# HBioquant/DiffBindFR

Hardware: AMD Instinct MI355X
Metric: poses_per_sec (higher is better)
Workload: dtype f32

## Files before the change

### diffbindfr_amd/csrc/api.cpp

```cpp
#include <cmath>
#include <cstdio>
#include <cstring>
#include <algorithm>
#include <atomic>
#include <map>

#include "common.h"

void launch_conv(const ConvArgs& a, hipStream_t st);
void launch_conv_layer(const ConvArgs* c4, hipStream_t st);
void launch_conv2(const Conv2Args& a, hipStream_t st);
void launch_conv2h(const Conv2Args& a, hipStream_t st);
void launch_convz(const ConvZArgs& a, hipStream_t st);
void launch_reduce_ln(const float* msg, const int* row_start, const int* row_cnt, int N, int D, const LNDesc& ln,
                      const float* old, int D_old, float* out, int ldo, int mode, hipStream_t st, const uint8_t* first = nullptr, unsigned long long sc_lanes = 0);
struct ReduceLayerArgs {
  const float* msg[4]; const int* row_start[4]; const int* row_cnt[4]; LNDesc ln[4];
  int NL, NA, D, D_old;
  const float* old_l; const float* old_a; float* out_l; float* out_a;
  const uint8_t* first[4]; unsigned long long sc_lanes[4];
};
static unsigned long long convz_sc_lanes(const ConvZ& z) {
  unsigned long long m = 0;
  for (int i = 0; i < z.n_io; ++i) m |= 0xfffull << (z.out_off[i] / 4);
// ... 5 lines not shown
  dbfr_batch b;
  const int* lig_batch; const int* atm_batch; const uint8_t* is_cab; const int* n_cab; const float* tr_sigma;
  float lig_cut2, atom_cut2, cross_cut2;
  int lig_cap, atom_cap, dynamic_cross;
  EdgeSet set[N_SETS];
  int* err;
  int step, lds_nl, lds_na, n_chunk, lanes;
};
void dbfr_edge_form(const dbfr_batch& b, int* n_chunk, int* lanes);
void launch_edges(const GraphArgs& A, bool heads_only, hipStream_t st);
void launch_edge_log(const GraphArgs& A, int* log_row, int stride, hipStream_t st);
void launch_edge_ties(const GraphArgs& A, int* log_row, int stride, float tol, hipStream_t st);
void launch_graph_chunks(const GraphArgs& A, hipStream_t st);
void launch_flat_chunks(const int* tgt, const int* n_edges, int max_edges, int span, int n_span, int* cnt0, int cap, int* chunk_es, int* chunk_gl, hipStream_t st);
void launch_row_absmax(const float* lx, const int* lig_ptr, float* out_l, const float* ax, const int* atm_ptr, float* out_a, int ld, int D, int G, int n_rows_a, hipStream_t st);
void launch_batch_vectors(const dbfr_batch& b, int* lig_batch, int* atm_batch, uint8_t* is_cab, int* n_cab,
                          int* tor_batch, int* sc_batch, hipStream_t st);
void launch_time_embed(const float* t, int G, float emb_scale, float* temb, hipStream_t st);
enum MlpIn { IN_LIGNODE = 0, IN_LIGEDGE = 1, IN_TG = 2, IN_G = 3 };
struct MlpArgs {
  Mlp2 w; int mode; const int* n_rows_dev; int n_rows_max; const float* temb; const int* row_graph_tab; const int* tgt;
  const int* aux; const float* dist; const float* bond_feat; int nfeat; const float* lig_node; int nnode;
  const float* gs_offset; const float* gs_coeff; float* out;
};
void launch_mlp(const MlpArgs& a, hipStream_t st);
struct AtomEncArgs {
  const float* pocket_feat; const int* atm_batch; const float* temb; const float* emb[5]; int dims[5];
  const float* lin_t; int NA; float* out;
};
void launch_atom_encoder(const AtomEncArgs& a, hipStream_t st);
void launch_center_edges(const dbfr_batch& b, int* tgt, int* gth, float* dist, float* sh, int* row_start, int* row_cnt,
                         hipStream_t st);
struct TrRotArgs {
  const float* gp; const float* temb; const float* tr_sigma; const float* rot_norm; Mlp2 tr, rot; int G;
  int scale_by_sigma; float* tr_out; float* rot_out; int* err;
};
void launch_trrot(const TrRotArgs& a, hipStream_t st);
void launch_bond_attr(const float* x, int ldx, const int* b0, const int* b1, const int* bsel, int stride, int n,
                      float* out, hipStream_t st);
void launch_tor_final(const float* feat, const Mlp2& w, const float* norm2, int scale, int n, float* out, hipStream_t st);
struct SdeLigArgs {
  dbfr_batch b; const float* tr_score; const float* rot_score; const float* tor_score; const float* z_tr;
  const float* z_rot; const float* z_tor; float dt, tr_g2, tr_gsdt, rot_g2, rot_gsdt, tor_g2, tor_gsdt; float* traj;
  int* err;
};
void launch_sde_ligand(const SdeLigArgs& a, hipStream_t st);
// ... 56 lines not shown

struct dbfr_model {
  dbfr_model_cfg cfg;
  std::vector<void*> allocs;
  ConvW layer[8][4];
  ConvW final_conv, tor_conv, sc_conv;
  ConvW2 layer2[8][4], tor_conv2, sc_conv2;
  ConvW2 layer2v[8][4];
  ConvZ layerz[8][4], tor_convz, sc_convz;
  int use_conv2;
  int gemm_split;
  int* queue;
  std::string fallback_convs;
  std::string rowscaled_convs;
  uint32_t layer_fallback;
  int* edge_log; int edge_log_steps, edge_log_graphs;
  int* tie_log; int tie_log_steps, tie_log_graphs; float tie_tol;
  Mlp2 lig_node_emb, lig_edge_emb, atom_edge_emb, la_edge_emb, center_edge_emb, tor_edge_emb, sc_edge_emb;
  Mlp2 tr_final, rot_final, tor_final, sc_final;
  const float* atom_emb[5]; int atom_dims[5];
  const float* atom_lin_t;
  const float *gs_lig_off, *gs_lig_c, *gs_atom_off, *gs_atom_c, *gs_cross_off, *gs_cross_c, *gs_center_off, *gs_center_c;
  int* a14_group;
  int profile;
  std::vector<hipEvent_t> ev;
  size_t ev_used;
  double* flops_dev;
  double fused_bytes_last;
  double executed_last;
  double useful_last;
  double form_bytes_last;
  double conv_ms_acc; int64_t conv_launches_acc;
};

template <typename T>
static T* upload(dbfr_model* m, const std::vector<T>& h, int* rc) {
  void* d = nullptr;
  size_t bytes = std::max<size_t>(h.size() * sizeof(T), 16);
  if (hipMalloc(&d, bytes) != hipSuccess) { *rc = DBFR_ERR_HIP; g_err = "hipMalloc failed (model weights)"; return nullptr; }
  if (!h.empty() && hipMemcpy(d, h.data(), h.size() * sizeof(T), hipMemcpyHostToDevice) != hipSuccess) {
    *rc = DBFR_ERR_HIP; g_err = "hipMemcpy failed (model weights)"; return nullptr;
  }
  m->allocs.push_back(d);
  return (T*)d;
}

typedef std::map<std::string, const dbfr_tensor*> TMap;

static const float* need(const TMap& tm, const std::string& name, int64_t numel, int* rc) {
  auto it = tm.find(name);
  if (it == tm.end()) { *rc = fail(DBFR_ERR_ARG, "missing tensor '" + name + "'"); return nullptr; }
  if (it->second->numel != numel) {
    *rc = fail(DBFR_ERR_ARG, "tensor '" + name + "' has " + std::to_string(it->second->numel) + " elements, expected " +
                                 std::to_string(numel));
    return nullptr;
  }
  return it->second->data;
}

static int pack_mlp(dbfr_model* m, const TMap& tm, const std::string& name, int in, int hid, int out, bool bias, Mlp2* o) {
  int rc = 0;
  const float* w0 = need(tm, name + ".lin.0.weight", (int64_t)hid * in, &rc);
  const float* w1 = need(tm, name + ".lin.3.weight", (int64_t)out * hid, &rc);
  const float *b0 = nullptr, *b1 = nullptr;
  if (bias) { b0 = need(tm, name + ".lin.0.bias", hid, &rc); b1 = need(tm, name + ".lin.3.bias", out, &rc); }
  if (rc) return rc;
  std::vector<float> w0t((size_t)in * hid), w1t((size_t)hid * out);
// ... 930 lines not shown
      acc(descs[i].n_edges, 2.0 * 144 * (144.0 + Ws[i]), m->flops_dev);
      acc(descs[i].n_edges, 4.0 * (Ws[i] + descs[i].w.D_in + 9) + 16.0, m->flops_dev + 1);
      acc(descs[i].n_edges, fused_bytes(descs[i].w.D_in, descs[i].w.D_out), m->flops_dev + 2);
      const double rows = 16.0 * descs[i].w.n_tiles;
      const bool f16 = (m->gemm_split >= DBFR_GEMM_SPLIT_F16 && !f16_fallback) || z;
      const double ex = f16 ? 3.0 * 2.0 * 144 * (144.0 + rows) : 2.0 * 144 * (144.0 + rows);
      if (!z || descs[i].w.n_tiles > 0) acc(descs[i].n_edges, ex, m->flops_dev + 3);
      if (!z) acc(descs[i].n_edges, ex, m->flops_dev + 4);
      else if (descs[i].w.n_tiles > 0) acc(descs[i].n_edges, 3.0 * 2.0 * 144 * rows, m->flops_dev + 4);
      const int D_in = descs[i].w.D_in, D_out = descs[i].w.D_out;
      const double in_bytes = 4.0 * (48 + 9 + 3 + 48 + 48 + D_in);
      if (!z) acc(descs[i].n_edges, fused_bytes(D_in, D_out), m->flops_dev + 5);
      else acc(descs[i].n_edges, in_bytes + 1.0 + (descs[i].w.n_tiles > 0 ? in_bytes + 4.0 * (D_out - 48 * z[i].w.n_io) : 0.0), m->flops_dev + 5);
    }
    launch_acc_batch(ab, st);
  }
}

static int run_score(dbfr_model* m, const dbfr_batch* B, const dbfr_cond* c, const dbfr_scores* out, Ws& w,
                     hipStream_t st, int step = 0) {
  const dbfr_model_cfg& cfg = m->cfg;
  const int G = B->G, NL = B->NL, NA = B->NA;
  launch_time_embed(c->t, G, cfg.emb_scale, w.temb, st);
  GraphArgs ga;
  ga.b = *B; ga.lig_batch = w.lig_batch; ga.atm_batch = w.atm_batch; ga.is_cab = w.is_cab; ga.n_cab = w.n_cab;
  ga.tr_sigma = c->tr_sigma;
  ga.lig_cut2 = cfg.lig_cutoff * cfg.lig_cutoff; ga.atom_cut2 = cfg.atom_cutoff * cfg.atom_cutoff;
  ga.cross_cut2 = cfg.dynamic_max_cross ? 1.0f : cfg.cross_cutoff * cfg.cross_cutoff;
  ga.lig_cap = cfg.lig_max_neighbors; ga.atom_cap = cfg.atom_max_neighbors; ga.dynamic_cross = cfg.dynamic_max_cross;
  for (int k = 0; k < N_SETS; ++k) ga.set[k] = w.set[k];
  ga.err = w.err; ga.step = step; ga.lds_nl = ga.lds_na = 0;
  dbfr_edge_form(*B, &ga.n_chunk, &ga.lanes);
  launch_edges(ga, false, st);
  if (int lrc = take_launch_error()) return lrc;
  if (m->gemm_split == DBFR_GEMM_REDUCE_FIRST) launch_graph_chunks(ga, st);
  if (m->edge_log && step < m->edge_log_steps) launch_edge_log(ga, m->edge_log + (size_t)step * N_SETS * m->edge_log_graphs, m->edge_log_graphs, st);
  if (m->tie_log && step < m->tie_log_steps) launch_edge_ties(ga, m->tie_log + (size_t)step * N_SETS * m->tie_log_graphs, m->tie_log_graphs, m->tie_tol, st);
  {
    MlpArgs a; memset(&a, 0, sizeof a);
    a.w = m->lig_node_emb; a.mode = IN_LIGNODE; a.n_rows_max = NL; a.temb = w.temb; a.row_graph_tab = w.lig_batch;
    a.lig_node = B->lig_node; a.nnode = cfg.lig_node_features; a.out = w.lig_x[0];
    launch_mlp(a, st);
  }
  {
    AtomEncArgs a; a.pocket_feat = B->pocket_feat; a.atm_batch = w.atm_batch; a.temb = w.temb;
    for (int i = 0; i < 5; ++i) { a.emb[i] = m->atom_emb[i]; a.dims[i] = m->atom_dims[i]; }
    a.lin_t = m->atom_lin_t; a.NA = NA; a.out = w.atom_x[0];
    launch_atom_encoder(a, st);
  }
  auto edge_mlp = [&](const Mlp2& mw, int mode, const EdgeSet& S, const int* tab, const float* off, const float* co) {
    MlpArgs a; memset(&a, 0, sizeof a);
    a.w = mw; a.mode = mode; a.n_rows_dev = S.n_edges; a.n_rows_max = S.cap; a.temb = w.temb; a.row_graph_tab = tab;
    a.tgt = S.tgt; a.aux = S.aux; a.dist = S.dist; a.bond_feat = B->bond_feat; a.nfeat = cfg.lig_edge_features;
    a.gs_offset = off; a.gs_coeff = co; a.out = S.emb;
    launch_mlp(a, st);
  };
  edge_mlp(m->lig_edge_emb, IN_LIGEDGE, w.set[SET_LL], w.lig_batch, m->gs_lig_off, m->gs_lig_c);
  edge_mlp(m->atom_edge_emb, IN_TG, w.set[SET_AA], w.atm_batch, m->gs_atom_off, m->gs_atom_c);
  edge_mlp(m->la_edge_emb, IN_TG, w.set[SET_AL], w.lig_batch, m->gs_cross_off, m->gs_cross_c);
  edge_mlp(m->la_edge_emb, IN_TG, w.set[SET_LA], w.atm_batch, m->gs_cross_off, m->gs_cross_c);
  static const int dims[4] = {48, 84, 120, 168};
  int cur = 0;
  for (int l = 0; l < cfg.num_conv_layers; ++l) {
    const int Di = dims[std::min(l, 3)], Do = dims[std::min(l + 1, 3)];
    const float *lx = w.lig_x[cur], *ax = w.atom_x[cur];
    float *lnew = w.lig_x[cur ^ 1], *anew = w.atom_x[cur ^ 1];
    const EdgeSet &LL = w.set[SET_LL], &AA = w.set[SET_AA], &AL = w.set[SET_AL], &LA = w.set[SET_LA];
    const ConvSite sites[4] = {conv_site(LL, G, lx, Di, LL.tgt, lx, Di, LL.gth, lx, Di, w.msg[0], w.xmax_l),
                               conv_site(AL, G, lx, Di, AL.tgt, ax, Di, AL.gth, ax, Di, w.msg[1], w.xmax_a),
                               conv_site(AA, G, ax, Di, AA.tgt, ax, Di, AA.gth, ax, Di, w.msg[2], w.xmax_a),
                               conv_site(LA, G, ax, Di, LA.tgt, lx, Di, LA.gth, lx, Di, w.msg[3], w.xmax_l)};
    const bool fallback = (m->layer_fallback >> l) & 1u;
    const bool rf = w.conv2 && m->gemm_split == DBFR_GEMM_REDUCE_FIRST && !fallback;
    if (w.conv2) {
      Conv2Desc ds[4]; ConvZDesc zs[4]; int Ws[4];
      for (int i = 0; i < 4; ++i) {
        ds[i] = conv2_desc(sites[i], rf ? m->layer2v[l][i] : m->layer2[l][i]);
// ... 12 lines not shown
      }
      launch_conv_layer(c4, st);
      if (m->profile == 1) (void)hipEventRecord(e1, st);
      if (m->profile)
        for (int i = 0; i < 4; ++i)
          launch_acc_flops(c4[i].n_edges, 2.0 * 144 * (144.0 + m->layer[l][i].W), 4.0 * (m->layer[l][i].W + Di + 9) + 16.0, fused_bytes(Di, Do), m->flops_dev, st);
    }
    ReduceLayerArgs ra;
    for (int i = 0; i < 4; ++i) {
      ra.msg[i] = sites[i].msg; ra.row_start[i] = sites[i].row_start; ra.row_cnt[i] = sites[i].row_cnt; ra.ln[i] = m->layer[l][i].ln;
      ra.first[i] = rf ? sites[i].seg_first : nullptr; ra.sc_lanes[i] = rf ? convz_sc_lanes(m->layerz[l][i]) : 0;
    }
    ra.NL = NL; ra.NA = NA; ra.D = Do; ra.D_old = Di; ra.old_l = lx; ra.old_a = ax; ra.out_l = lnew; ra.out_a = anew;
    launch_reduce_ln_layer(ra, st);
    cur ^= 1;
  }
  const int D = dims[std::min(cfg.num_conv_layers, 3)];
  if (D != MAXD) return fail(DBFR_ERR_ARG, "heads need num_conv_layers >= 3");
  const float *lx = w.lig_x[cur], *ax = w.atom_x[cur];
  launch_center_edges(*B, w.c_tgt, w.c_gth, w.c_dist, w.c_sh, w.c_row_start, w.c_row_cnt, st);
  {
    MlpArgs a; memset(&a, 0, sizeof a);
    a.w = m->center_edge_emb; a.mode = IN_TG; a.n_rows_max = NL; a.temb = w.temb; a.row_graph_tab = w.lig_batch;
    a.dist = w.c_dist; a.gs_offset = m->gs_center_off; a.gs_coeff = m->gs_center_c; a.out = w.c_emb;
    launch_mlp(a, st);
  }
  conv_call(m, m->final_conv, flat_site(w.n_edges6 + 7, NL, w.c_tgt, w.c_gth, w.c_emb, w.c_sh, lx, D, w.c_gth, nullptr, 0, w.c_gth, lx, D, w.msg[0]), st);
  launch_reduce_ln(w.msg[0], w.c_row_start, w.c_row_cnt, G, 12, m->final_conv.ln, nullptr, 0, w.gp, 12, 2, st);
  {
    TrRotArgs a; a.gp = w.gp; a.temb = w.temb; a.tr_sigma = c->tr_sigma; a.rot_norm = c->rot_score_norm;
    a.tr = m->tr_final; a.rot = m->rot_final; a.G = G; a.scale_by_sigma = cfg.scale_by_sigma; a.tr_out = out->tr;
    a.rot_out = out->rot; a.err = w.err;
    launch_trrot(a, st);
  }
  struct TorHead {
    bool on; int n; const EdgeSet* S; ConvSite site;
    const float* nodes; const int *b0, *b1, *bsel; int stride; float* attr;
    const Mlp2* emb; const float *gs_off, *gs_c;
    const ConvW* cw; const ConvW2* cw2; const ConvZ* cz;
    const Mlp2* fin; const float* norm2; float *feat, *out;
  };
  const EdgeSet &T = w.set[SET_TOR], &S = w.set[SET_SC];
  TorHead heads[2];
  {
    TorHead& h = heads[0];
    h.on = B->NTOR > 0; h.n = B->NTOR; h.S = &T;
    h.site = conv_site(T, G, lx, D, T.gth, w.tor_attr, NS, T.tgt, lx, D, w.msg[0], w.xmax_l);
// ... 378 lines not shown
  const ConvW* cw = pick_conv(m, layer, family);
  if (!cw) return fail(DBFR_ERR_ARG, "no such conv");
  unsigned long long lanes = 0;
  if (seg_first) {
    if (layer == -1 || cw->K != 144) return fail(DBFR_ERR_ARG, "dbfr_test_reduce_ln2: seg_first with a conv that has no reduce-first form");
    lanes = convz_sc_lanes(*pick_conv144(m, layer, family).z);
  }
  launch_reduce_ln(msg, row_start, row_cnt, n_nodes, cw->D_out, cw->ln, old, d_old, out, cw->D_out, mode, (hipStream_t)hip_stream, seg_first, lanes);
  HIPCHECK(hipGetLastError());
  return DBFR_OK;
}

extern "C" int dbfr_test_reduce_ln(dbfr_model* m, int32_t layer, int32_t family, const float* msg,
                                   const int32_t* row_start, const int32_t* row_cnt, int32_t n_nodes, const float* old,
                                   int32_t d_old, float* out, int32_t mode, void* hip_stream) {
  if (!m) return fail(DBFR_ERR_ARG, "null model");
  const ConvW* cw = pick_conv(m, layer, family);
  if (!cw) return fail(DBFR_ERR_ARG, "no such conv");
  launch_reduce_ln(msg, row_start, row_cnt, n_nodes, cw->D_out, cw->ln, old, d_old, out, cw->D_out, mode,
                   (hipStream_t)hip_stream);
  HIPCHECK(hipGetLastError());
  return DBFR_OK;
}
```

### diffbindfr_amd/csrc/conv.hip

```cpp
#include <cstdio>
#include <cstdlib>
#include <type_traits>
#include <vector>

#include "common.h"

#ifndef CONV_PRIO
#define CONV_PRIO 0
#endif
#ifndef CONV_XPF
#define CONV_XPF 0
#endif
#ifndef CONV_NB2_WAVES
#define CONV_NB2_WAVES 2
#endif
#define XS_LD (MAXD + 4)

typedef float f32x4 __attribute__((ext_vector_type(4)));

#define TRACE_BLOCKS 1024
#define TRACE_TILES 48
#define TRACE_REC (2 + 3 * TRACE_TILES + 8)
#define RSTAMP(k) do { if ((ABL & 16) && a.trace && bid < TRACE_BLOCKS && lane == 0) a.trace[((size_t)bid * 4 + wave) * TRACE_REC + 2 + 3 * TRACE_TILES + (k)] = __builtin_amdgcn_s_memrealtime(); } while (0)
#define TSTAMP(k) do { if ((ABL & 16) && a.trace && bid < TRACE_BLOCKS && lane == 0) a.trace[((size_t)bid * 4 + wave) * TRACE_REC + 2 + 3 * TRACE_TILES + (k)] = __builtin_readcyclecounter(); } while (0)
// ... 500 lines not shown
      float v = buf[wave][c];
      float* o = out + (size_t)node * ldo + c;
      if (mode == 0) v = (c < D_old ? old[(size_t)node * D_old + c] : 0.f) + v;
      else if (mode == 1) v = *o + v;
      *o = v;
    }
  }
}

void launch_reduce_ln(const float* msg, const int* row_start, const int* row_cnt, int N, int D, const LNDesc& ln,
                      const float* old, int D_old, float* out, int ldo, int mode, hipStream_t st, const uint8_t* first, unsigned long long sc_lanes) {
  if (N <= 0) return;
  hipLaunchKernelGGL(k_reduce_ln, dim3((N + 3) / 4), dim3(256), 0, st, msg, row_start, row_cnt, N, D, ln, old, D_old,
                     out, ldo, mode, first, sc_lanes);
}

struct ReduceLayerArgs {
  const float* msg[4]; const int* row_start[4]; const int* row_cnt[4]; LNDesc ln[4];
  int NL, NA, D, D_old;
  const float* old_l; const float* old_a; float* out_l; float* out_a;
  const uint8_t* first[4]; unsigned long long sc_lanes[4];
};

__device__ __forceinline__ void mean_ln(const float* __restrict__ msg, int rs, int rc, int D, const LNDesc& ln, float* bw, int lane, const uint8_t* first, unsigned long long sc_lanes) {
  const int d4 = D >> 2;
  const f32x4 acc = row_sum(msg, rs, rc, D, lane, first, sc_lanes);
  if (lane < d4) {
    const float cntf = (float)max(rc, 1);
    bw[4 * lane] = acc[0] / cntf; bw[4 * lane + 1] = acc[1] / cntf; bw[4 * lane + 2] = acc[2] / cntf; bw[4 * lane + 3] = acc[3] / cntf;
  }
  __builtin_amdgcn_wave_barrier();
  int iw = 0, ib = 0;
  for (int bk = 0; bk < ln.nblk; ++bk) {
    const int mul = ln.mul[bk], dim = ln.dim[bk], off = ln.off[bk];
    const int nel = mul * dim;
    float mean[3] = {0.f, 0.f, 0.f};
    const bool d3 = dim == 3;
    for (int i = lane; i < nel; i += 64) {
      int comp = d3 ? i % 3 : 0;
      float v = bw[off + i];
      if (comp == 0) mean[0] += v; else if (comp == 1) mean[1] += v; else mean[2] += v;
    }
    for (int o = 32; o > 0; o >>= 1) mean[0] += __shfl_xor(mean[0], o);
    mean[0] /= (float)mul;
    if (d3) {
#pragma unroll
      for (int c = 1; c < 3; ++c) {
        for (int o = 32; o > 0; o >>= 1) mean[c] += __shfl_xor(mean[c], o);
        mean[c] /= (float)mul;
      }
    }
    float sq = 0.f;
    for (int i = lane; i < nel; i += 64) {
      int u = d3 ? i / 3 : i, comp = d3 ? i - 3 * u : 0;
      float v = bw[off + i] - (comp == 0 ? mean[0] : comp == 1 ? mean[1] : mean[2]) * ln.mean_shift[iw + u];
      bw[off + i] = v;
      sq += v * v;
    }
    __builtin_amdgcn_wave_barrier();
    for (int o = 32; o > 0; o >>= 1) sq += __shfl_xor(sq, o);
    const float inv = 1.0f / sqrtf(sq / (float)nel + 1e-5f);
    for (int i = lane; i < nel; i += 64) {
      int u = d3 ? i / 3 : i;
      float v = bw[off + i] * (inv * ln.weight[iw + u]);
      if (ln.is0e[bk]) v += ln.bias[ib + u];
      bw[off + i] = v;
    }
    iw += mul;
    if (ln.is0e[bk]) ib += mul;
  }
  __builtin_amdgcn_wave_barrier();
}

__global__ __launch_bounds__(256) void k_reduce_ln_layer(ReduceLayerArgs a) {
  __shared__ float buf[4][2][MAXD];
  const int lane = threadIdx.x & 63, wave = threadIdx.x >> 6;
  const int nbl = (a.NL + 3) / 4;
  const bool lig = (int)blockIdx.x < nbl;
  const int node = (lig ? blockIdx.x : blockIdx.x - nbl) * 4 + wave;
  const int N = lig ? a.NL : a.NA;
  if (node >= N) return;
  const int s0 = lig ? 0 : 2;
  mean_ln(a.msg[s0], a.row_start[s0][node], a.row_cnt[s0][node], a.D, a.ln[s0], buf[wave][0], lane, a.first[s0], a.sc_lanes[s0]);
  mean_ln(a.msg[s0 + 1], a.row_start[s0 + 1][node], a.row_cnt[s0 + 1][node], a.D, a.ln[s0 + 1], buf[wave][1], lane, a.first[s0 + 1], a.sc_lanes[s0 + 1]);
  const float* old = (lig ? a.old_l : a.old_a) + (size_t)node * a.D_old;
  float* out = (lig ? a.out_l : a.out_a) + (size_t)node * a.D;
#pragma unroll
  for (int j = 0; j < 3; ++j) {
    const int c = lane + 64 * j;
    if (c < a.D) out[c] = ((c < a.D_old ? old[c] : 0.f) + buf[wave][0][c]) + buf[wave][1][c];
  }
}

void launch_reduce_ln_layer(const ReduceLayerArgs& a, hipStream_t st) {
  const int nb = (a.NL + 3) / 4 + (a.NA + 3) / 4;
  if (nb <= 0) return;
  hipLaunchKernelGGL(k_reduce_ln_layer, dim3(nb), dim3(256), 0, st, a);
}
```

### diffbindfr_amd/csrc/graph.hip

```cpp
#include "common.h"

#define MAX_NL 256
#define MAX_NA 8192

enum SetKind { SET_LL = 0, SET_AA = 1, SET_AL = 2, SET_LA = 3, SET_TOR = 4, SET_SC = 5, N_SETS = 6 };

struct GraphArgs {
  dbfr_batch b;
  const int* lig_batch;
  const int* atm_batch;
  const uint8_t* is_cab;
  const int* n_cab;
  const float* tr_sigma;
  float lig_cut2, atom_cut2, cross_cut2;
  int lig_cap, atom_cap, dynamic_cross;
  EdgeSet set[N_SETS];
  int* err;
  int step;
  int lds_nl, lds_na;
  int n_chunk;
  int lanes;
};

__device__ __forceinline__ float d2_rn(float ax, float ay, float az, float bx, float by, float bz) {
// ... 648 lines not shown
void launch_time_embed(const float* t, int G, float emb_scale, float* temb, hipStream_t st) {
  hipLaunchKernelGGL(k_time_embed, dim3((G * EMB + 255) / 256), dim3(256), 0, st, t, G, emb_scale, temb);
}

enum MlpIn { IN_LIGNODE = 0, IN_LIGEDGE = 1, IN_TG = 2, IN_G = 3 };

struct MlpArgs {
  Mlp2 w;
  int mode;
  const int* n_rows_dev;
  int n_rows_max;
  const float* temb;
  const int* row_graph_tab;
  const int* tgt;
  const int* aux;
  const float* dist;
  const float* bond_feat;
  int nfeat;
  const float* lig_node;
  int nnode;
  const float* gs_offset;
  const float* gs_coeff;
  float* out;
};

#define MLP_ROWS 64
#define MLP_MAXIN 80

__global__ __launch_bounds__(256) void k_mlp(MlpArgs a) {
  __shared__ float xin[MLP_ROWS][MLP_MAXIN + 1];
  __shared__ float hid[MLP_ROWS][NS + 1];
  __shared__ float w0[MLP_MAXIN * NS];
  __shared__ float w1[NS * NS];
  __shared__ float s_gs[EMB];
  const int nrows = a.n_rows_dev ? min(*a.n_rows_dev, a.n_rows_max) : a.n_rows_max;
  if ((int)blockIdx.x * MLP_ROWS >= nrows) return;
  const int in = a.w.in;
  for (int i = threadIdx.x; i < in * NS; i += 256) w0[i] = a.w.w0t[i];
  for (int i = threadIdx.x; i < NS * NS; i += 256) w1[i] = a.w.w1t[i];
  const float coeff = a.gs_coeff ? a.gs_coeff[0] : 0.f;
  if (threadIdx.x < EMB) s_gs[threadIdx.x] = a.gs_offset ? a.gs_offset[threadIdx.x] : 0.f;
  __syncthreads();
  const int kin = (in + 3) & ~3;
  if (kin > in)
    for (int i = threadIdx.x; i < (kin - in) * NS; i += 256) w0[in * NS + i] = 0.f;
  typedef float f32x4 __attribute__((ext_vector_type(4)));
// ... 47 lines not shown
  }
#pragma unroll
  for (int t = 0; t < 3; ++t)
#pragma unroll
    for (int r = 0; r < 4; ++r) hid[row][16 * t + 4 * g + r] = fmaxf(acc[t][r], 0.f);
  __syncthreads();
#pragma unroll
  for (int t = 0; t < 3; ++t)
#pragma unroll
    for (int r = 0; r < 4; ++r) acc[t][r] = a.w.b1 ? a.w.b1[16 * t + 4 * g + r] : 0.f;
#pragma unroll
  for (int k = 0; k < NS; k += 4) {
    const float bv = hid[row][k + g];
#pragma unroll
    for (int t = 0; t < 3; ++t) acc[t] = __builtin_amdgcn_mfma_f32_16x16x4f32(w1[(k + g) * NS + 16 * t + n], bv, acc[t], 0, 0, 0);
  }
  if (row < nr) {
#pragma unroll
    for (int t = 0; t < 3; ++t) *reinterpret_cast<f32x4*>(a.out + (size_t)(r0 + row) * NS + 16 * t + 4 * g) = acc[t];
  }
  }
}

void launch_mlp(const MlpArgs& a, hipStream_t st) {
  if (a.n_rows_max <= 0) return;
  const int tiles = (a.n_rows_max + MLP_ROWS - 1) / MLP_ROWS;
  hipLaunchKernelGGL(k_mlp, dim3(tiles < 1024 ? tiles : 1024), dim3(256), 0, st, a);
}

struct AtomEncArgs {
  const float* pocket_feat;
  const int* atm_batch;
  const float* temb;
  const float* emb[5];
  int dims[5];
  const float* lin_t;
  int NA;
  float* out;
};

__global__ __launch_bounds__(256) void k_atom_encoder(AtomEncArgs a) {
  __shared__ float w[(NS + EMB) * NS];
  __shared__ float x[16][NS + EMB];
  for (int i = threadIdx.x; i < (NS + EMB) * NS; i += 256) w[i] = a.lin_t[i];
  const int r0 = blockIdx.x * 16;
  for (int i = threadIdx.x; i < 16 * (NS + EMB); i += 256) {
    int r = i / (NS + EMB), c = i % (NS + EMB);
    int row = r0 + r;
// ... 30 lines not shown
```

### diffbindfr_amd/lib.py

```python
import ctypes as C
import os

HERE = os.path.dirname(os.path.abspath(__file__))
LIB_PATH = os.environ.get("DBFR_LIB") or os.path.join(HERE, "libdbfr.so")

DBFR_OK = 0
DBFR_ERR_CAPACITY = -3
ERRORS = {-1: "DBFR_ERR_ARG", -2: "DBFR_ERR_HIP", -3: "DBFR_ERR_CAPACITY", -4: "DBFR_ERR_SELFTEST",
          -5: "DBFR_ERR_NUMERIC"}

i32, f32, vp = C.c_int32, C.c_float, C.c_void_p


class ModelCfg(C.Structure):
    _fields_ = [(n, i32) for n in ("ns", "nv", "sh_lmax", "num_conv_layers", "lig_node_features",
                                   "lig_edge_features", "distance_embed_dim", "sigma_embed_dim")] + \
               [(n, f32) for n in ("emb_scale", "lig_cutoff", "atom_cutoff", "cross_cutoff", "center_max_distance")] + \
               [(n, i32) for n in ("atom_max_neighbors", "lig_max_neighbors", "dynamic_max_cross", "scale_by_sigma",
                                   "no_sc_torsion")]


class Tensor(C.Structure):
    _fields_ = [("name", C.c_char_p), ("data", vp), ("numel", C.c_int64)]

# ... 232 lines not shown

class XtcOpts(C.Structure):
    _fields_ = [("precision", f32), ("dt", f32), ("first_step", i32), ("box", f32 * 9)]


class SitesOpts(C.Structure):
    _fields_ = [(n, f32) for n in ("spacing", "probe", "ray_length", "lining_cutoff")] + \
               [(n, i32) for n in ("min_buried", "min_points", "max_sites")]


class SitesIn(C.Structure):
    _fields_ = [("n_prot", i32), ("n_res", i32), ("max_points", C.c_int64)] + \
               [(n, vp) for n in ("res_ptr", "aatype", "atom37_pos", "atom37_mask", "radius")]


class SitesOut(C.Structure):
    _fields_ = [(n, vp) for n in ("n_sites", "label", "n_points", "score", "idx_sum", "centre", "lining", "grid", "occupancy",
                                  "burial", "labels")]


SYMBOLS = ["dbfr_model_create", "dbfr_model_destroy", "dbfr_model_set_edge_log", "dbfr_model_set_tie_log", "dbfr_model_fallback_convs", "dbfr_model_rowscaled_convs", "dbfr_model_set_gemm", "dbfr_model_get_gemm", "dbfr_workspace_bytes", "dbfr_score", "dbfr_sample",
           "dbfr_sample_range", "dbfr_capacity_report",
           "dbfr_init_poses", "dbfr_extract_templates", "dbfr_status_sync", "dbfr_abi_version", "dbfr_build_id", "dbfr_last_error", "dbfr_wigner3j", "dbfr_conv_paths", "dbfr_test_pack_f16_tiles", "dbfr_test_pack_f16_rows", "dbfr_test_chunk_table", "dbfr_test_pack_f16_depth", "dbfr_probe_mfma_f16",
           "dbfr_profile_enable", "dbfr_profile_read", "dbfr_profile_fused_bytes", "dbfr_profile_executed_flops", "dbfr_profile_useful_flops", "dbfr_workspace_layout", "dbfr_test_conv", "dbfr_test_conv2", "dbfr_test_reduce_ln", "dbfr_test_reduce_ln2", "dbfr_test_sde_step",
           "dbfr_pose_metrics", "dbfr_pdb_format", "dbfr_pdb_write_files", "dbfr_select_pocket", "dbfr_sdf_format",
           "dbfr_sdf_write_files", "dbfr_mdn_model_create", "dbfr_mdn_model_destroy", "dbfr_mdn_workspace_bytes", "dbfr_mdn_forward", "dbfr_mdn_pocket_features",
           "dbfr_vina_workspace_bytes", "dbfr_vina_score", "dbfr_vina_score_at", "dbfr_vina_minimize",
           "dbfr_vina_flex_workspace_bytes", "dbfr_vina_flex_score_at", "dbfr_vina_flex_minimize",
           "dbfr_pose_rmsd_matrix", "dbfr_select_modes", "dbfr_pose_check",
           "dbfr_pdb_atom_map", "dbfr_complex_pdb_format", "dbfr_complex_pdb_write_files", "dbfr_xtc_workspace_bytes", "dbfr_xtc_encode",
           "dbfr_sites_workspace_bytes", "dbfr_find_sites", "dbfr_interactions", "dbfr_pocket_check", "dbfr_sasa",
           "dbfr_seq_align", "dbfr_holo_site", "dbfr_holo_metrics", "dbfr_hetero_check", "dbfr_hydrogens"]

_lib = None


class DbfrError(RuntimeError):
    pass


def load():
    global _lib
    if _lib is not None:
        return _lib
    if not os.path.exists(LIB_PATH):
        raise DbfrError(f"{LIB_PATH} is missing: build the HIP library first "
                        f"(python -m diffbindfr_amd.build). There is no CPU fallback.")
# ... 20 lines not shown
    lib.dbfr_init_poses.argtypes = [vp, C.POINTER(Batch), C.POINTER(InitTape), vp, vp]
    lib.dbfr_extract_templates.argtypes = [i32, vp, vp, vp, vp, vp, vp, vp, vp]
    lib.dbfr_status_sync.argtypes = [vp, vp, C.POINTER(C.c_int64)]
    lib.dbfr_wigner3j.argtypes = [i32, i32, i32, C.POINTER(C.c_double)]
    lib.dbfr_conv_paths.argtypes = [i32, C.POINTER(i32), i32, C.POINTER(i32)]
    lib.dbfr_test_pack_f16_tiles.argtypes = [vp, vp, i32, vp, C.POINTER(i32)]
    lib.dbfr_test_pack_f16_depth.argtypes = [vp, vp, i32, C.POINTER(i32), C.POINTER(i32)]
    lib.dbfr_test_pack_f16_rows.argtypes = [vp, vp, i32, vp, C.POINTER(i32), vp, C.POINTER(i32)]
    lib.dbfr_test_chunk_table.argtypes = [vp, vp, i32, i32, vp, i32, vp, vp, vp]
    lib.dbfr_probe_mfma_f16.argtypes = [C.c_double, C.POINTER(C.c_double), vp]
    lib.dbfr_profile_enable.argtypes = [vp, i32]
    lib.dbfr_profile_fused_bytes.argtypes = [vp, C.POINTER(C.c_double)]
    lib.dbfr_profile_executed_flops.argtypes = [vp, C.POINTER(C.c_double)]
    lib.dbfr_profile_useful_flops.argtypes = [vp, C.POINTER(C.c_double), C.POINTER(C.c_double)]
    lib.dbfr_profile_read.argtypes = [vp, C.POINTER(C.c_double), C.POINTER(C.c_int64), C.POINTER(C.c_double),
                                      C.POINTER(C.c_double), i32]
    lib.dbfr_workspace_layout.argtypes = [vp, C.POINTER(Batch), C.POINTER(Limits), C.c_char_p, C.c_size_t,
                                          C.POINTER(C.c_size_t), C.POINTER(C.c_size_t), i32]
    lib.dbfr_test_conv.argtypes = [vp, i32, i32, i32, vp, vp, vp, vp, vp, vp, i32, vp, vp, i32, vp, vp, i32, vp, vp]
    lib.dbfr_test_conv2.argtypes = lib.dbfr_test_conv.argtypes
    lib.dbfr_test_reduce_ln.argtypes = [vp, i32, i32, vp, vp, vp, i32, vp, i32, vp, i32, vp]
    lib.dbfr_test_reduce_ln2.argtypes = [vp, i32, i32, vp, vp, vp, i32, vp, i32, vp, i32, vp, vp]
    lib.dbfr_test_sde_step.argtypes = [vp, C.POINTER(Batch), C.POINTER(Step), C.POINTER(Scores), C.POINTER(Noise), vp, vp, vp]
    lib.dbfr_select_pocket.argtypes = [i32, i32, vp, i32, vp, vp, vp, vp, C.c_double, i32, vp, vp, vp]
    lib.dbfr_pose_metrics.argtypes = [C.POINTER(PoseMetricsIn), C.POINTER(PoseMetricsOut), vp]
    lib.dbfr_pdb_format.argtypes = [C.POINTER(PdbTopology), i32, vp, vp, i32, i32, vp, C.c_int64]
    lib.dbfr_pdb_format.restype = C.c_int64
    lib.dbfr_pdb_write_files.argtypes = [C.POINTER(PdbTopology), i32, vp, vp, i32, C.POINTER(C.c_char_p), i32]
    lib.dbfr_sdf_format.argtypes = [C.POINTER(SdfTemplate), vp, vp, C.c_int64]
    lib.dbfr_sdf_format.restype = C.c_int64
    lib.dbfr_sdf_write_files.argtypes = [C.POINTER(SdfTemplate), vp, i32, C.POINTER(C.c_char_p), i32]
    lib.dbfr_mdn_model_create.argtypes = [C.POINTER(Tensor), i32, C.POINTER(vp)]
    lib.dbfr_mdn_model_destroy.argtypes = [vp]
    lib.dbfr_mdn_model_destroy.restype = None
    lib.dbfr_mdn_workspace_bytes.argtypes = [C.POINTER(MdnBatch), C.POINTER(C.c_size_t)]
    lib.dbfr_mdn_pocket_features.argtypes = [i32, i32, vp, vp, vp, vp, i32, vp, vp, vp, vp, vp, vp, vp, vp]
    lib.dbfr_mdn_forward.argtypes = [vp, C.POINTER(MdnBatch), vp, vp, vp, vp, C.c_size_t, vp]
    lib.dbfr_vina_workspace_bytes.argtypes = [C.POINTER(VinaIn), C.POINTER(C.c_size_t)]
    lib.dbfr_vina_score.argtypes = [C.POINTER(VinaIn), vp, vp, vp, vp, C.c_size_t, vp]
    lib.dbfr_vina_score_at.argtypes = [C.POINTER(VinaIn), vp, vp, vp, vp, vp, vp, vp, C.c_size_t, vp]
    lib.dbfr_vina_minimize.argtypes = [C.POINTER(VinaIn), C.POINTER(VinaOpts), vp, vp, vp, vp, C.c_size_t, vp]
    lib.dbfr_vina_flex_workspace_bytes.argtypes = [C.POINTER(VinaFlexIn), C.POINTER(C.c_size_t)]
    lib.dbfr_vina_flex_score_at.argtypes = [C.POINTER(VinaFlexIn), vp, vp, vp, vp, vp, vp, vp, vp, vp, vp, C.c_size_t, vp]
    lib.dbfr_vina_flex_minimize.argtypes = [C.POINTER(VinaFlexIn), C.POINTER(VinaOpts), vp, vp, vp, vp, vp, vp, C.c_size_t, vp]
    lib.dbfr_pose_rmsd_matrix.argtypes = [C.POINTER(PoseRmsdIn), vp, vp]
    lib.dbfr_select_modes.argtypes = [C.POINTER(PoseRmsdIn), vp, vp, C.POINTER(ModesOpts), vp, vp, vp, vp]
# ... 44 lines not shown
```

### include/dbfr.h

```cpp
#ifndef DBFR_H
#define DBFR_H

#include <stddef.h>
#include <stdint.h>

#ifdef __cplusplus
extern "C" {
#endif

#define DBFR_ABI_VERSION 7

typedef enum {
  DBFR_OK = 0,
  DBFR_ERR_ARG = -1,
  DBFR_ERR_HIP = -2,
  DBFR_ERR_CAPACITY = -3,
  DBFR_ERR_SELFTEST = -4,
  DBFR_ERR_NUMERIC = -5
} dbfr_status;

typedef struct dbfr_model dbfr_model;

typedef struct {
  int32_t ns, nv, sh_lmax;
// ... 825 lines not shown
int dbfr_probe_mfma_f16(double seconds, double* tflops, void* hip_stream);

int dbfr_workspace_layout(const dbfr_model* m, const dbfr_batch* b, const dbfr_limits* lim, char* names,
                          size_t names_cap, size_t* offsets, size_t* bytes, int32_t max_entries);

int dbfr_test_conv(dbfr_model* m, int32_t layer, int32_t family, int32_t n_edges, const int32_t* n_edges_dev,
                   const int32_t* tgt, const int32_t* gth, const float* emb, const float* sh, const float* tab1,
                   int32_t ld1, const int32_t* idx1, const float* tab2, int32_t ld2, const int32_t* idx2,
                   const float* x, int32_t ldx, float* msg, void* hip_stream);
int dbfr_test_conv2(dbfr_model* m, int32_t layer, int32_t family, int32_t n_edges, const int32_t* n_edges_dev,
                    const int32_t* tgt, const int32_t* gth, const float* emb, const float* sh, const float* tab1,
                    int32_t ld1, const int32_t* idx1, const float* tab2, int32_t ld2, const int32_t* idx2,
                    const float* x, int32_t ldx, float* msg, void* hip_stream);
int dbfr_test_reduce_ln(dbfr_model* m, int32_t layer, int32_t family, const float* msg, const int32_t* row_start,
                        const int32_t* row_cnt, int32_t n_nodes, const float* old, int32_t d_old, float* out,
                        int32_t mode, void* hip_stream);
int dbfr_test_reduce_ln2(dbfr_model* m, int32_t layer, int32_t family, const float* msg, const int32_t* row_start,
                         const int32_t* row_cnt, int32_t n_nodes, const float* old, int32_t d_old, float* out,
                         int32_t mode, const uint8_t* seg_first, void* hip_stream);

int dbfr_test_sde_step(const dbfr_model* m, const dbfr_batch* b, const dbfr_step* step, const dbfr_scores* scores,
                       const dbfr_noise* z, float* atom14_out, int32_t* err_word_out, void* hip_stream);

#ifdef __cplusplus
}
#endif
#endif
```

Measured before the change: 519.4.

## Factor per-graph time-embedding term out of edge MLPs and use MFMA; DPP wave reductions

Edge-embedding MLPs whose input concatenates the time embedding with a Gaussian distance expansion now compute the time-embedding half of the first layer once per graph in a small prefix kernel. A new MFMA-based kernel then adds that prefix per row and evaluates only the distance half plus the second layer, with weights held in registers. This removes redundant per-edge work on the shared time-embedding input. The layer mean/layernorm reduction also swaps shfl_xor butterflies for permlane-swap and DPP reductions and hoists the row sums. These changes add a lazily grown device buffer, a CU-count query, and new test entry points.

```diff
diff --git a/diffbindfr_amd/csrc/api.cpp b/diffbindfr_amd/csrc/api.cpp
--- a/diffbindfr_amd/csrc/api.cpp
+++ b/diffbindfr_amd/csrc/api.cpp
@@ -51,6 +51,7 @@
   Mlp2 w; int mode; const int* n_rows_dev; int n_rows_max; const float* temb; const int* row_graph_tab; const int* tgt;
   const int* aux; const float* dist; const float* bond_feat; int nfeat; const float* lig_node; int nnode;
   const float* gs_offset; const float* gs_coeff; float* out;
+  float* prefix; int n_graphs;
 };
 void launch_mlp(const MlpArgs& a, hipStream_t st);
 struct AtomEncArgs {
@@ -153,6 +154,7 @@
   const float* atom_lin_t;
   const float *gs_lig_off, *gs_lig_c, *gs_atom_off, *gs_atom_c, *gs_cross_off, *gs_cross_c, *gs_center_off, *gs_center_c;
   int* a14_group;
+  float* mlp_prefix; int mlp_prefix_graphs;
   int profile;
   std::vector<hipEvent_t> ev;
   size_t ev_used;
@@ -174,6 +176,20 @@
   }
   m->allocs.push_back(d);
   return (T*)d;
+}
+
+static float* mlp_prefix_buf(dbfr_model* m, int G) {
+  if (G <= m->mlp_prefix_graphs) return m->mlp_prefix;
+  void* d = nullptr;
+  if (hipMalloc(&d, (size_t)G * NS * sizeof(float)) != hipSuccess) { g_err = "hipMalloc failed (embedding-MLP prefix)"; return nullptr; }
+  if (m->mlp_prefix) {
+    for (void*& p : m->allocs) if (p == (void*)m->mlp_prefix) p = d;
+    (void)hipFree(m->mlp_prefix);
+  } else {
+    m->allocs.push_back(d);
+  }
+  m->mlp_prefix = (float*)d; m->mlp_prefix_graphs = G;
+  return m->mlp_prefix;
 }
 
 typedef std::map<std::string, const dbfr_tensor*> TMap;
@@ -1150,6 +1166,8 @@
   const dbfr_model_cfg& cfg = m->cfg;
   const int G = B->G, NL = B->NL, NA = B->NA;
   launch_time_embed(c->t, G, cfg.emb_scale, w.temb, st);
+  float* const mlp_prefix = mlp_prefix_buf(m, G);
+  if (!mlp_prefix) return DBFR_ERR_HIP;
   GraphArgs ga;
   ga.b = *B; ga.lig_batch = w.lig_batch; ga.atm_batch = w.atm_batch; ga.is_cab = w.is_cab; ga.n_cab = w.n_cab;
   ga.tr_sigma = c->tr_sigma;
@@ -1180,7 +1198,7 @@
     MlpArgs a; memset(&a, 0, sizeof a);
     a.w = mw; a.mode = mode; a.n_rows_dev = S.n_edges; a.n_rows_max = S.cap; a.temb = w.temb; a.row_graph_tab = tab;
     a.tgt = S.tgt; a.aux = S.aux; a.dist = S.dist; a.bond_feat = B->bond_feat; a.nfeat = cfg.lig_edge_features;
-    a.gs_offset = off; a.gs_coeff = co; a.out = S.emb;
+    a.gs_offset = off; a.gs_coeff = co; a.out = S.emb; a.prefix = mlp_prefix; a.n_graphs = G;
     launch_mlp(a, st);
   };
   edge_mlp(m->lig_edge_emb, IN_LIGEDGE, w.set[SET_LL], w.lig_batch, m->gs_lig_off, m->gs_lig_c);
@@ -1239,7 +1257,7 @@
   {
     MlpArgs a; memset(&a, 0, sizeof a);
     a.w = m->center_edge_emb; a.mode = IN_TG; a.n_rows_max = NL; a.temb = w.temb; a.row_graph_tab = w.lig_batch;
-    a.dist = w.c_dist; a.gs_offset = m->gs_center_off; a.gs_coeff = m->gs_center_c; a.out = w.c_emb;
+    a.dist = w.c_dist; a.gs_offset = m->gs_center_off; a.gs_coeff = m->gs_center_c; a.out = w.c_emb; a.prefix = mlp_prefix; a.n_graphs = G;
     launch_mlp(a, st);
   }
   conv_call(m, m->final_conv, flat_site(w.n_edges6 + 7, NL, w.c_tgt, w.c_gth, w.c_emb, w.c_sh, lx, D, w.c_gth, nullptr, 0, w.c_gth, lx, D, w.msg[0]), st);
@@ -1664,3 +1682,47 @@
   HIPCHECK(hipGetLastError());
   return DBFR_OK;
 }
+
+extern "C" int dbfr_test_mlp(dbfr_model* m, int32_t which, int32_t n_rows_max, const int32_t* n_rows_dev, const float* temb, int32_t n_graphs,
+                             const int32_t* row_graph_tab, const int32_t* tgt, const int32_t* aux, const float* dist, const float* bond_feat,
+                             const float* lig_node, float* out, void* hip_stream) {
+  if (!m || !out || which < 0 || which > 6 || n_rows_max < 0 || n_graphs <= 0) return fail(DBFR_ERR_ARG, "dbfr_test_mlp: bad argument");
+  const Mlp2* ws[7] = {&m->lig_node_emb, &m->lig_edge_emb, &m->atom_edge_emb, &m->la_edge_emb, &m->center_edge_emb, &m->tor_edge_emb, &m->sc_edge_emb};
+  const int modes[7] = {IN_LIGNODE, IN_LIGEDGE, IN_TG, IN_TG, IN_TG, IN_G, IN_G};
+  const float* offs[7] = {nullptr, m->gs_lig_off, m->gs_atom_off, m->gs_cross_off, m->gs_center_off, m->gs_lig_off, m->gs_atom_off};
+  const float* cos[7] = {nullptr, m->gs_lig_c, m->gs_atom_c, m->gs_cross_c, m->gs_center_c, m->gs_lig_c, m->gs_atom_c};
+  const int mode = modes[which];
+  if (which == 6 && m->cfg.no_sc_torsion) return fail(DBFR_ERR_ARG, "dbfr_test_mlp: the model has no side-chain torsion head");
+  if ((mode != IN_G && (!temb || !row_graph_tab)) || (mode != IN_LIGNODE && !dist) || (mode == IN_LIGNODE && !lig_node) ||
+      (mode == IN_LIGEDGE && (!aux || !bond_feat || !tgt)))
+    return fail(DBFR_ERR_ARG, "dbfr_test_mlp: an array the mode reads is null");
+  MlpArgs a; memset(&a, 0, sizeof a);
+  a.w = *ws[which]; a.mode = mode; a.n_rows_dev = n_rows_dev; a.n_rows_max = n_rows_max; a.temb = temb; a.row_graph_tab = row_graph_tab;
+  a.tgt = tgt; a.aux = aux; a.dist = dist; a.bond_feat = bond_feat; a.nfeat = m->cfg.lig_edge_features; a.lig_node = lig_node;
+  a.nnode = m->cfg.lig_node_features; a.gs_offset = offs[which]; a.gs_coeff = cos[which]; a.out = out;
+  a.n_graphs = n_graphs;
+  if (mode == IN_TG && !(a.prefix = mlp_prefix_buf(m, n_graphs))) return DBFR_ERR_HIP;
+  launch_mlp(a, (hipStream_t)hip_stream);
+  HIPCHECK(hipGetLastError());
+  return DBFR_OK;
+}
+
+extern "C" int dbfr_test_reduce_ln_layer(dbfr_model* m, int32_t layer, const float* const* msg, const int32_t* const* row_start,
+                                         const int32_t* const* row_cnt, int32_t n_lig, int32_t n_atm, const float* old_l, const float* old_a,
+                                         int32_t d_old, float* out_l, float* out_a, const uint8_t* const* seg_first, void* hip_stream) {
+  if (!m || !msg || !row_start || !row_cnt || layer < 0 || layer >= m->cfg.num_conv_layers || n_lig < 0 || n_atm < 0)
+    return fail(DBFR_ERR_ARG, "dbfr_test_reduce_ln_layer: bad argument");
+  ReduceLayerArgs ra;
+  ra.D = m->layer[layer][0].D_out;
+  if (d_old < 0 || d_old > ra.D || (n_lig > 0 && (!old_l || !out_l)) || (n_atm > 0 && (!old_a || !out_a)))
+    return fail(DBFR_ERR_ARG, "dbfr_test_reduce_ln_layer: bad node arrays");
+  for (int i = 0; i < 4; ++i) {
+    if (!msg[i] || !row_start[i] || !row_cnt[i]) return fail(DBFR_ERR_ARG, "dbfr_test_reduce_ln_layer: null edge-set array");
+    ra.msg[i] = msg[i]; ra.row_start[i] = row_start[i]; ra.row_cnt[i] = row_cnt[i]; ra.ln[i] = m->layer[layer][i].ln;
+    ra.first[i] = seg_first ? seg_first[i] : nullptr; ra.sc_lanes[i] = seg_first ? convz_sc_lanes(m->layerz[layer][i]) : 0;
+  }
+  ra.NL = n_lig; ra.NA = n_atm; ra.D_old = d_old; ra.old_l = old_l; ra.old_a = old_a; ra.out_l = out_l; ra.out_a = out_a;
+  launch_reduce_ln_layer(ra, (hipStream_t)hip_stream);
+  HIPCHECK(hipGetLastError());
+  return DBFR_OK;
+}
diff --git a/diffbindfr_amd/csrc/conv.hip b/diffbindfr_amd/csrc/conv.hip
--- a/diffbindfr_amd/csrc/conv.hip
+++ b/diffbindfr_amd/csrc/conv.hip
@@ -546,9 +546,45 @@
   const uint8_t* first[4]; unsigned long long sc_lanes[4];
 };
 
-__device__ __forceinline__ void mean_ln(const float* __restrict__ msg, int rs, int rc, int D, const LNDesc& ln, float* bw, int lane, const uint8_t* first, unsigned long long sc_lanes) {
+__device__ __forceinline__ float xadd_swap32(float v) {
+  const auto r = __builtin_amdgcn_permlane32_swap(__float_as_uint(v), __float_as_uint(v), false, false);
+  return __uint_as_float(r[0]) + __uint_as_float(r[1]);
+}
+__device__ __forceinline__ float xadd_swap16(float v) {
+  const auto r = __builtin_amdgcn_permlane16_swap(__float_as_uint(v), __float_as_uint(v), false, false);
+  return __uint_as_float(r[0]) + __uint_as_float(r[1]);
+}
+template <int CTRL>
+__device__ __forceinline__ float dpp_mov(float v) {
+  return __uint_as_float((unsigned)__builtin_amdgcn_update_dpp(0, (int)__float_as_uint(v), CTRL, 0xf, 0xf, false));
+}
+#define DPP_ROW_ROR8 0x128
+#define DPP_ROW_HALF_MIRROR 0x141
+#define DPP_QUAD_3210 0x1b
+#define DPP_QUAD_2301 0x4e
+#define DPP_QUAD_1032 0xb1
+__device__ __forceinline__ float xadd_step(float v, int o) {
+  switch (o) {
+    case 32: return xadd_swap32(v);
+    case 16: return xadd_swap16(v);
+    case 8: return v + dpp_mov<DPP_ROW_ROR8>(v);
+    case 4: return v + dpp_mov<DPP_QUAD_3210>(dpp_mov<DPP_ROW_HALF_MIRROR>(v));
+    case 2: return v + dpp_mov<DPP_QUAD_2301>(v);
+    default: return v + dpp_mov<DPP_QUAD_1032>(v);
+  }
+}
+__device__ __forceinline__ float wave_sum(float v) {
+#pragma unroll
+  for (int o = 32; o > 0; o >>= 1) v = xadd_step(v, o);
+  return v;
+}
+__device__ __forceinline__ void wave_sum3(float& a, float& b, float& c) {
+#pragma unroll
+  for (int o = 32; o > 0; o >>= 1) { a = xadd_step(a, o); b = xadd_step(b, o); c = xadd_step(c, o); }
+}
+
+__device__ __forceinline__ void mean_ln(const f32x4 acc, int rc, int D, const LNDesc& ln, float* bw, int lane) {
   const int d4 = D >> 2;
-  const f32x4 acc = row_sum(msg, rs, rc, D, lane, first, sc_lanes);
   if (lane < d4) {
     const float cntf = (float)max(rc, 1);
     bw[4 * lane] = acc[0] / cntf; bw[4 * lane + 1] = acc[1] / cntf; bw[4 * lane + 2] = acc[2] / cntf; bw[4 * lane + 3] = acc[3] / cntf;
@@ -565,14 +601,12 @@
       float v = bw[off + i];
       if (comp == 0) mean[0] += v; else if (comp == 1) mean[1] += v; else mean[2] += v;
     }
-    for (int o = 32; o > 0; o >>= 1) mean[0] += __shfl_xor(mean[0], o);
-    mean[0] /= (float)mul;
     if (d3) {
-#pragma unroll
-      for (int c = 1; c < 3; ++c) {
-        for (int o = 32; o > 0; o >>= 1) mean[c] += __shfl_xor(mean[c], o);
-        mean[c] /= (float)mul;
-      }
+      wave_sum3(mean[0], mean[1], mean[2]);
+      mean[0] /= (float)mul; mean[1] /= (float)mul; mean[2] /= (float)mul;
+    } else {
+      mean[0] = wave_sum(mean[0]);
+      mean[0] /= (float)mul;
     }
     float sq = 0.f;
     for (int i = lane; i < nel; i += 64) {
@@ -582,7 +616,7 @@
       sq += v * v;
     }
     __builtin_amdgcn_wave_barrier();
-    for (int o = 32; o > 0; o >>= 1) sq += __shfl_xor(sq, o);
+    sq = wave_sum(sq);
     const float inv = 1.0f / sqrtf(sq / (float)nel + 1e-5f);
     for (int i = lane; i < nel; i += 64) {
       int u = d3 ? i / 3 : i;
@@ -604,9 +638,12 @@
   const int node = (lig ? blockIdx.x : blockIdx.x - nbl) * 4 + wave;
   const int N = lig ? a.NL : a.NA;
   if (node >= N) return;
-  const int s0 = lig ? 0 : 2;
-  mean_ln(a.msg[s0], a.row_start[s0][node], a.row_cnt[s0][node], a.D, a.ln[s0], buf[wave][0], lane, a.first[s0], a.sc_lanes[s0]);
-  mean_ln(a.msg[s0 + 1], a.row_start[s0 + 1][node], a.row_cnt[s0 + 1][node], a.D, a.ln[s0 + 1], buf[wave][1], lane, a.first[s0 + 1], a.sc_lanes[s0 + 1]);
+  const int s0 = lig ? 0 : 2, s1 = s0 + 1;
+  const int rs0 = a.row_start[s0][node], rc0 = a.row_cnt[s0][node], rs1 = a.row_start[s1][node], rc1 = a.row_cnt[s1][node];
+  const f32x4 acc0 = row_sum(a.msg[s0], rs0, rc0, a.D, lane, a.first[s0], a.sc_lanes[s0]);
+  mean_ln(acc0, rc0, a.D, a.ln[s0], buf[wave][0], lane);
+  const f32x4 acc1 = row_sum(a.msg[s1], rs1, rc1, a.D, lane, a.first[s1], a.sc_lanes[s1]);
+  mean_ln(acc1, rc1, a.D, a.ln[s1], buf[wave][1], lane);
   const float* old = (lig ? a.old_l : a.old_a) + (size_t)node * a.D_old;
   float* out = (lig ? a.out_l : a.out_a) + (size_t)node * a.D;
 #pragma unroll
diff --git a/diffbindfr_amd/csrc/graph.hip b/diffbindfr_amd/csrc/graph.hip
--- a/diffbindfr_amd/csrc/graph.hip
+++ b/diffbindfr_amd/csrc/graph.hip
@@ -694,6 +694,8 @@
   const float* gs_offset;
   const float* gs_coeff;
   float* out;
+  float* prefix;
+  int n_graphs;
 };
 
 #define MLP_ROWS 64
@@ -787,8 +789,135 @@
   }
 }
 
+#define MLPT_LD 52
+#define MLPT_J0 (EMB / 4)
+#define MLPT_J1 (2 * EMB / 4)
+#define MLPT_J2 (NS / 4)
+#define MLPT_WGS_PER_CU 4
+typedef float mlp_f32x4 __attribute__((ext_vector_type(4)));
+
+__global__ __launch_bounds__(64) void k_mlp_prefix(MlpArgs a) {
+  const int lane = threadIdx.x, n = lane & 15, g = lane >> 4;
+  const int graph = blockIdx.x * 16 + n;
+  const int gr = min(graph, a.n_graphs - 1);
+  mlp_f32x4 acc[3];
+#pragma unroll
+  for (int t = 0; t < 3; ++t)
+#pragma unroll
+    for (int r = 0; r < 4; ++r) acc[t][r] = a.w.b0 ? a.w.b0[16 * t + 4 * g + r] : 0.f;
+#pragma unroll
+  for (int j = 0; j < MLPT_J0; ++j) {
+    const float bv = a.temb[gr * EMB + 4 * j + g];
+#pragma unroll
+    for (int t = 0; t < 3; ++t) acc[t] = __builtin_amdgcn_mfma_f32_16x16x4f32(a.w.w0t[(4 * j + g) * NS + 16 * t + n], bv, acc[t], 0, 0, 0);
+  }
+  if (graph < a.n_graphs) {
+#pragma unroll
+    for (int t = 0; t < 3; ++t) *reinterpret_cast<mlp_f32x4*>(a.prefix + (size_t)graph * NS + 16 * t + 4 * g) = acc[t];
+  }
+}
+
+template <bool TG>
+__global__ __launch_bounds__(256) void k_mlp_tg(MlpArgs a) {
+  __shared__ float patch[4][16][MLPT_LD];
+  const int nrows = a.n_rows_dev ? min(*a.n_rows_dev, a.n_rows_max) : a.n_rows_max;
+  const int nblk = (nrows + 15) >> 4;
+  const int lane = threadIdx.x & 63, wave = threadIdx.x >> 6, n = lane & 15, g = lane >> 4;
+  const int wave0 = blockIdx.x * 4 + wave, nwaves = gridDim.x * 4;
+  if (wave0 >= nblk) return;
+  float w0f[MLPT_J1 - MLPT_J0][3], w1f[MLPT_J2][3], off[MLPT_J1 - MLPT_J0], b1v[3][4], b0v[3][4];
+#pragma unroll
+  for (int j = 0; j < MLPT_J1 - MLPT_J0; ++j) {
+#pragma unroll
+    for (int t = 0; t < 3; ++t) w0f[j][t] = a.w.w0t[(4 * (j + (TG ? MLPT_J0 : 0)) + g) * NS + 16 * t + n];
+    off[j] = a.gs_offset[4 * j + g];
+  }
+#pragma unroll
+  for (int j = 0; j < MLPT_J2; ++j)
+#pragma unroll
+    for (int t = 0; t < 3; ++t) w1f[j][t] = a.w.w1t[(4 * j + g) * NS + 16 * t + n];
+#pragma unroll
+  for (int t = 0; t < 3; ++t)
+#pragma unroll
+    for (int r = 0; r < 4; ++r) {
+      b1v[t][r] = a.w.b1 ? a.w.b1[16 * t + 4 * g + r] : 0.f;
+      b0v[t][r] = !TG && a.w.b0 ? a.w.b0[16 * t + 4 * g + r] : 0.f;
+    }
+  const float coeff = a.gs_coeff[0], last = a.gs_offset[EMB - 1];
+  float* pw = &patch[wave][n][0];
+  for (int blk = wave0; blk < nblk; blk += nwaves) {
+    const int row = 16 * blk + n;
+    const bool live = row < nrows;
+    const int arow = live ? row : nrows - 1;
+    const float dcl = fminf(a.dist[arow], last);
+    mlp_f32x4 acc[3];
+    if (TG) {
+      const int gph = a.row_graph_tab[a.tgt ? a.tgt[arow] : arow];
+#pragma unroll
+      for (int t = 0; t < 3; ++t) acc[t] = *reinterpret_cast<const mlp_f32x4*>(a.prefix + (size_t)gph * NS + 16 * t + 4 * g);
+    } else {
+#pragma unroll
+      for (int t = 0; t < 3; ++t)
+#pragma unroll
+        for (int r = 0; r < 4; ++r) acc[t][r] = b0v[t][r];
+    }
+#pragma unroll
+    for (int j = 0; j < MLPT_J1 - MLPT_J0; ++j) {
+      const float d = dcl - off[j];
+      const float bv = expf(coeff * (d * d));
+#pragma unroll
+      for (int t = 0; t < 3; ++t) acc[t] = __builtin_amdgcn_mfma_f32_16x16x4f32(w0f[j][t], bv, acc[t], 0, 0, 0);
+    }
+#pragma unroll
+    for (int t = 0; t < 3; ++t) {
+      mlp_f32x4 h;
+#pragma unroll
+      for (int r = 0; r < 4; ++r) h[r] = fmaxf(acc[t][r], 0.f);
+      *reinterpret_cast<mlp_f32x4*>(pw + 16 * t + 4 * g) = h;
+    }
+    __builtin_amdgcn_wave_barrier();
+    float hb[MLPT_J2];
+#pragma unroll
+    for (int j = 0; j < MLPT_J2; ++j) hb[j] = pw[4 * j + g];
+    __builtin_amdgcn_wave_barrier();
+#pragma unroll
+    for (int t = 0; t < 3; ++t)
+#pragma unroll
+      for (int r = 0; r < 4; ++r) acc[t][r] = b1v[t][r];
+#pragma unroll
+    for (int j = 0; j < MLPT_J2; ++j)
+#pragma unroll
+      for (int t = 0; t < 3; ++t) acc[t] = __builtin_amdgcn_mfma_f32_16x16x4f32(w1f[j][t], hb[j], acc[t], 0, 0, 0);
+    if (live) {
+#pragma unroll
+      for (int t = 0; t < 3; ++t) *reinterpret_cast<mlp_f32x4*>(a.out + (size_t)row * NS + 16 * t + 4 * g) = acc[t];
+    }
+  }
+}
+
+static int mlp_device_cus() {
+  static int cus[64] = {0};
+  int dev = 0;
+  if (hipGetDevice(&dev) != hipSuccess || dev < 0 || dev >= 64) return 256;
+  if (!cus[dev]) {
+    int n = 0;
+    cus[dev] = (hipDeviceGetAttribute(&n, hipDeviceAttributeMultiprocessorCount, dev) == hipSuccess && n > 0) ? n : 256;
+  }
+  return cus[dev];
+}
+
 void launch_mlp(const MlpArgs& a, hipStream_t st) {
   if (a.n_rows_max <= 0) return;
+  const int wgs = (a.n_rows_max + 63) / 64, cap = MLPT_WGS_PER_CU * mlp_device_cus();
+  if (a.mode == IN_TG && a.prefix && a.w.in == 2 * EMB && a.gs_offset && a.gs_coeff && a.dist) {
+    hipLaunchKernelGGL(k_mlp_prefix, dim3((a.n_graphs + 15) / 16), dim3(64), 0, st, a);
+    hipLaunchKernelGGL(k_mlp_tg<true>, dim3(wgs < cap ? wgs : cap), dim3(256), 0, st, a);
+    return;
+  }
+  if (a.mode == IN_G && a.w.in == EMB && a.gs_offset && a.gs_coeff && a.dist) {
+    hipLaunchKernelGGL(k_mlp_tg<false>, dim3(wgs < cap ? wgs : cap), dim3(256), 0, st, a);
+    return;
+  }
   const int tiles = (a.n_rows_max + MLP_ROWS - 1) / MLP_ROWS;
   hipLaunchKernelGGL(k_mlp, dim3(tiles < 1024 ? tiles : 1024), dim3(256), 0, st, a);
 }
diff --git a/diffbindfr_amd/lib.py b/diffbindfr_amd/lib.py
--- a/diffbindfr_amd/lib.py
+++ b/diffbindfr_amd/lib.py
@@ -278,7 +278,7 @@
 SYMBOLS = ["dbfr_model_create", "dbfr_model_destroy", "dbfr_model_set_edge_log", "dbfr_model_set_tie_log", "dbfr_model_fallback_convs", "dbfr_model_rowscaled_convs", "dbfr_model_set_gemm", "dbfr_model_get_gemm", "dbfr_workspace_bytes", "dbfr_score", "dbfr_sample",
            "dbfr_sample_range", "dbfr_capacity_report",
            "dbfr_init_poses", "dbfr_extract_templates", "dbfr_status_sync", "dbfr_abi_version", "dbfr_build_id", "dbfr_last_error", "dbfr_wigner3j", "dbfr_conv_paths", "dbfr_test_pack_f16_tiles", "dbfr_test_pack_f16_rows", "dbfr_test_chunk_table", "dbfr_test_pack_f16_depth", "dbfr_probe_mfma_f16",
-           "dbfr_profile_enable", "dbfr_profile_read", "dbfr_profile_fused_bytes", "dbfr_profile_executed_flops", "dbfr_profile_useful_flops", "dbfr_workspace_layout", "dbfr_test_conv", "dbfr_test_conv2", "dbfr_test_reduce_ln", "dbfr_test_reduce_ln2", "dbfr_test_sde_step",
+           "dbfr_profile_enable", "dbfr_profile_read", "dbfr_profile_fused_bytes", "dbfr_profile_executed_flops", "dbfr_profile_useful_flops", "dbfr_workspace_layout", "dbfr_test_conv", "dbfr_test_conv2", "dbfr_test_reduce_ln", "dbfr_test_reduce_ln2", "dbfr_test_sde_step", "dbfr_test_mlp", "dbfr_test_reduce_ln_layer",
            "dbfr_pose_metrics", "dbfr_pdb_format", "dbfr_pdb_write_files", "dbfr_select_pocket", "dbfr_sdf_format",
            "dbfr_sdf_write_files", "dbfr_mdn_model_create", "dbfr_mdn_model_destroy", "dbfr_mdn_workspace_bytes", "dbfr_mdn_forward", "dbfr_mdn_pocket_features",
            "dbfr_vina_workspace_bytes", "dbfr_vina_score", "dbfr_vina_score_at", "dbfr_vina_minimize",
@@ -345,6 +345,8 @@
     lib.dbfr_test_reduce_ln.argtypes = [vp, i32, i32, vp, vp, vp, i32, vp, i32, vp, i32, vp]
     lib.dbfr_test_reduce_ln2.argtypes = [vp, i32, i32, vp, vp, vp, i32, vp, i32, vp, i32, vp, vp]
     lib.dbfr_test_sde_step.argtypes = [vp, C.POINTER(Batch), C.POINTER(Step), C.POINTER(Scores), C.POINTER(Noise), vp, vp, vp]
+    lib.dbfr_test_mlp.argtypes = [vp, i32, i32, vp, vp, i32, vp, vp, vp, vp, vp, vp, vp, vp]
+    lib.dbfr_test_reduce_ln_layer.argtypes = [vp, i32, vp, vp, vp, i32, i32, vp, vp, i32, vp, vp, vp, vp]
     lib.dbfr_select_pocket.argtypes = [i32, i32, vp, i32, vp, vp, vp, vp, C.c_double, i32, vp, vp, vp]
     lib.dbfr_pose_metrics.argtypes = [C.POINTER(PoseMetricsIn), C.POINTER(PoseMetricsOut), vp]
     lib.dbfr_pdb_format.argtypes = [C.POINTER(PdbTopology), i32, vp, vp, i32, i32, vp, C.c_int64]
diff --git a/include/dbfr.h b/include/dbfr.h
--- a/include/dbfr.h
+++ b/include/dbfr.h
@@ -871,6 +871,13 @@
 int dbfr_test_sde_step(const dbfr_model* m, const dbfr_batch* b, const dbfr_step* step, const dbfr_scores* scores,
                        const dbfr_noise* z, float* atom14_out, int32_t* err_word_out, void* hip_stream);
 
+int dbfr_test_mlp(dbfr_model* m, int32_t which, int32_t n_rows_max, const int32_t* n_rows_dev, const float* temb, int32_t n_graphs,
+                  const int32_t* row_graph_tab, const int32_t* tgt, const int32_t* aux, const float* dist, const float* bond_feat,
+                  const float* lig_node, float* out, void* hip_stream);
+int dbfr_test_reduce_ln_layer(dbfr_model* m, int32_t layer, const float* const* msg, const int32_t* const* row_start,
+                              const int32_t* const* row_cnt, int32_t n_lig, int32_t n_atm, const float* old_l, const float* old_a,
+                              int32_t d_old, float* out_l, float* out_a, const uint8_t* const* seg_first, void* hip_stream);
+
 #ifdef __cplusplus
 }
 #endif
```

Result: slower. 474.1 (-8.7%).
